# jteutenberg/downpore

Measured on AMD Instinct MI355X. Metric: overlaps/sec (all-vs-all PAF), higher is better.
Workload: dtype u64

## Files before the change

downpore_amd/csrc/dp_kbuild.hip:

```cpp
#include <algorithm>
#include <cstdio>
#include <cstdlib>
#include <cstring>

#include "dp_common.h"

typedef unsigned long long kb_u64;

#define KB_TILE 16384
#define KB_THREADS 1024
#define KB_P3_CAP 8192

struct KbGeom {
    int k, b1, b2, r;
    int pbits, rbits;
    uint32_t dlo, dhi;
};

struct KbBuf {
    uint32_t* lo;
    void* hi;
    int hb;
};
__device__ __forceinline__ kb_u64 kb_ld(const KbBuf B, kb_u64 i) {
    if (B.hb == 8) return ((const kb_u64*)B.lo)[i];
    kb_u64 v = B.lo[i];
    if (B.hb == 1) v |= (kb_u64)((const uint8_t*)B.hi)[i] << 32;
    else if (B.hb == 2) v |= (kb_u64)((const uint16_t*)B.hi)[i] << 32;
    else if (B.hb == 4) v |= (kb_u64)((const uint32_t*)B.hi)[i] << 32;
    return v;
}
__device__ __forceinline__ void kb_st(const KbBuf B, kb_u64 i, kb_u64 v) {
    if (B.hb == 8) {
        ((kb_u64*)B.lo)[i] = v;
        return;
    }
    B.lo[i] = (uint32_t)v;
    if (B.hb == 1) ((uint8_t*)B.hi)[i] = (uint8_t)(v >> 32);
    else if (B.hb == 2) ((uint16_t*)B.hi)[i] = (uint16_t)(v >> 32);
    else if (B.hb == 4) ((uint32_t*)B.hi)[i] = (uint32_t)(v >> 32);
}

__global__ void kb_group_table(const uint64_t* __restrict__ boff, uint32_t n_reads, uint32_t* __restrict__ gread) {
    const uint32_t r = blockIdx.x * blockDim.x + threadIdx.x;
    if (r >= n_reads) return;
    const uint64_t a0 = boff[r] * 4, a1 = boff[r + 1] * 4;
    for (uint64_t j = (a0 + 1023) >> 10; (j << 10) < a1; j++) gread[j] = r;
}

__device__ __forceinline__ uint32_t kb_read_of(uint64_t a, const uint32_t* __restrict__ gread, const uint64_t* __restrict__ boff) {
    uint32_t r = gread[a >> 10];
    while (boff[r + 1] * 4 <= a) r++;
    return r;
}

__device__ __forceinline__ uint32_t kb_load16(const uint8_t* __restrict__ packed, const uint64_t* __restrict__ boff,
                                              const uint32_t* __restrict__ len, const uint32_t* __restrict__ gread, uint64_t n_groups,
                                              uint64_t g, int half, int k, uint32_t kmer[16], uint32_t* read_out = nullptr,
                                              uint64_t* start_out = nullptr) {
    if (g >= n_groups) return 0u;
    const uint64_t a = g * 32 + (uint64_t)half * 16;
    const uint32_t r = kb_read_of(g * 32, gread, boff);
    const uint32_t L = len[r];
    if (L < (uint32_t)k) return 0u;
    const uint64_t a0 = boff[r] * 4, a1 = a0 + (L - k + 1);
    if (read_out) *read_out = r;
    if (start_out) *start_out = a0;
    if (a >= a1) return 0u;
    const uint32_t* p = (const uint32_t*)(packed + g * 8) + half;
    const uint32_t w0 = __builtin_bswap32(p[0]), w1 = __builtin_bswap32(p[1]);
    const int sh = 32 - 2 * k;
    uint32_t mask = 0;
#pragma unroll
    for (int j = 0; j < 16; j++) {
        const uint32_t win = j ? __builtin_amdgcn_alignbit(w0, w1, 32 - 2 * j) : w0;
        kmer[j] = win >> sh;
        if (a + j >= a0 && a + j < a1) mask |= 1u << j;
    }
    return mask;
}

__global__ __launch_bounds__(KB_THREADS) void kb_count1(const uint8_t* __restrict__ packed, const uint64_t* __restrict__ boff,
                                                        const uint32_t* __restrict__ len, const uint32_t* __restrict__ gread,
                                                        uint64_t n_groups, KbGeom G, kb_u64* __restrict__ cnt1) {
    __shared__ uint32_t hist[1024];
    const int nb = 1 << G.b1;
    for (int i = threadIdx.x; i < nb; i += KB_THREADS) hist[i] = 0;
    __syncthreads();
    const int dsh = 2 * G.k - G.b1;
    const uint64_t tiles = (n_groups * 2 + KB_THREADS - 1) / KB_THREADS;
    for (uint64_t t = blockIdx.x; t < tiles; t += gridDim.x) {
        const uint64_t h = t * KB_THREADS + threadIdx.x;
        uint32_t kmer[16];
        const uint32_t m = kb_load16(packed, boff, len, gread, n_groups, h >> 1, (int)(h & 1), G.k, kmer);
#pragma unroll
        for (int j = 0; j < 16; j++)
            if ((m >> j) & 1) atomicAdd(&hist[kmer[j] >> dsh], 1u);
    }
    __syncthreads();
    for (int i = threadIdx.x; i < nb; i += KB_THREADS)
        if (hist[i]) atomicAdd(&cnt1[i], (kb_u64)hist[i]);
}

template <int E>
__device__ __forceinline__ void kb_tile_out(const kb_u64 (&e)[E], uint32_t m, int dshift, uint32_t dmask, uint32_t* hist ,
                                            uint32_t* lstart , kb_u64* gbase , kb_u64* sorted ,
                                            kb_u64* __restrict__ cursor, const KbBuf out) {
    const int nb = (int)dmask + 1;
    for (int i = threadIdx.x; i < nb; i += KB_THREADS) hist[i] = 0;
    __syncthreads();
    uint32_t rk[E];
#pragma unroll
    for (int j = 0; j < E; j++) rk[j] = ((m >> j) & 1) ? atomicAdd(&hist[(uint32_t)(e[j] >> dshift) & dmask], 1u) : 0u;
    __syncthreads();
    {
        const int per = (nb + KB_THREADS - 1) / KB_THREADS;
        uint32_t loc[4] = {0, 0, 0, 0}, s = 0;
        for (int u = 0; u < per; u++) {
            const int b = threadIdx.x * per + u;
            loc[u] = b < nb ? hist[b] : 0u;
            s += loc[u];
        }
        const int lane = dp_lane(), wave = threadIdx.x >> 6;
        __shared__ uint32_t wsum[KB_THREADS / 64];
        uint32_t x = (uint32_t)wave_incl_sum((int)s);
        if (lane == 63) wsum[wave] = x;
        __syncthreads();
        uint32_t base = x - s;
        for (int w = 0; w < wave; w++) base += wsum[w];
        for (int u = 0; u < per; u++) {
            const int b = threadIdx.x * per + u;
            if (b < nb) {
                lstart[b] = base;
                if (loc[u]) gbase[b] = atomicAdd(&cursor[b], (kb_u64)loc[u]);
                base += loc[u];
            }
        }
    }
    __syncthreads();
    uint32_t total = 0;
#pragma unroll
    for (int j = 0; j < E; j++)
        if ((m >> j) & 1) {
            const uint32_t d = (uint32_t)(e[j] >> dshift) & dmask;
            sorted[lstart[d] + rk[j]] = e[j];
        }
    __syncthreads();
    total = lstart[nb - 1] + hist[nb - 1];
    for (uint32_t i = threadIdx.x; i < total; i += KB_THREADS) {
        const kb_u64 v = sorted[i];
        const uint32_t d = (uint32_t)(v >> dshift) & dmask;
        kb_st(out, gbase[d] + (kb_u64)(i - lstart[d]), v);
    }
    __syncthreads();
}

__global__ __launch_bounds__(KB_THREADS) void kb_part1(const uint8_t* __restrict__ packed, const uint64_t* __restrict__ boff,
                                                       const uint32_t* __restrict__ len, const uint32_t* __restrict__ gread,
                                                       uint64_t n_groups, KbGeom G, kb_u64* __restrict__ cursor, const KbBuf out) {
    __shared__ uint32_t hist[1024], lstart[1024];
    __shared__ kb_u64 gbase[1024];
    __shared__ kb_u64 sorted[KB_TILE];
    const int pay = G.pbits + G.rbits;
    const int dsh = pay + 2 * G.k - G.b1;
    const uint32_t dmask = (1u << G.b1) - 1u;
    const uint64_t tiles = (n_groups * 2 + KB_THREADS - 1) / KB_THREADS;
    for (uint64_t t = blockIdx.x; t < tiles; t += gridDim.x) {
        const uint64_t h = t * KB_THREADS + threadIdx.x;
        uint32_t kmer[16], rd = 0;
        uint64_t a0 = 0;
        const uint32_t m = kb_load16(packed, boff, len, gread, n_groups, h >> 1, (int)(h & 1), G.k, kmer, &rd, &a0);
        kb_u64 e[16];
        const kb_u64 a = (h >> 1) * 32 + (h & 1) * 16;
        const kb_u64 low = ((kb_u64)rd << G.pbits) + (a - a0);
        uint32_t mine = m;
        const int ksh = 2 * G.k - G.b1;
#pragma unroll
        for (int j = 0; j < 16; j++) {
            e[j] = ((kb_u64)kmer[j] << pay) | (low + (kb_u64)j);
            const uint32_t d = kmer[j] >> ksh;
            if (d < G.dlo || d >= G.dhi) mine &= ~(1u << j);
        }
        kb_tile_out<16>(e, mine, dsh, dmask, hist, lstart, gbase, sorted, cursor, out);
    }
}

__device__ __forceinline__ uint32_t kb_bucket_of_tile(const uint32_t* __restrict__ tile_start, int nb1, uint32_t t) {
    int lo = 0, hi = nb1;
    while (hi - lo > 1) {
        const int mid = (lo + hi) >> 1;
        if (tile_start[mid] <= t) lo = mid;
        else hi = mid;
    }
    return (uint32_t)lo;
}

__global__ __launch_bounds__(KB_THREADS) void kb_count2(const KbBuf in, const kb_u64* __restrict__ base1,
                                                        const uint32_t* __restrict__ tile_start, KbGeom G, kb_u64* __restrict__ cnt2) {
    __shared__ uint32_t hist[1024];
    const int nb1 = 1 << G.b1, nb2 = 1 << G.b2;
    const uint32_t n_tiles = tile_start[nb1];
    const int dsh = G.pbits + G.rbits + 2 * G.k - G.b1 - G.b2;
    const uint32_t dmask = (uint32_t)nb2 - 1u;
    for (uint32_t t = blockIdx.x; t < n_tiles; t += gridDim.x) {
        const uint32_t b = kb_bucket_of_tile(tile_start, nb1, t);
        const kb_u64 lo = base1[b] + (kb_u64)(t - tile_start[b]) * KB_TILE, hi = min(base1[b + 1], lo + KB_TILE);
        for (int i = threadIdx.x; i < nb2; i += KB_THREADS) hist[i] = 0;
        __syncthreads();
        for (kb_u64 i = lo + threadIdx.x; i < hi; i += KB_THREADS) atomicAdd(&hist[(uint32_t)(kb_ld(in, i) >> dsh) & dmask], 1u);
        __syncthreads();
        for (int i = threadIdx.x; i < nb2; i += KB_THREADS)
            if (hist[i]) atomicAdd(&cnt2[(kb_u64)b * nb2 + i], (kb_u64)hist[i]);
        __syncthreads();
    }
}

__global__ __launch_bounds__(KB_THREADS) void kb_part2(const KbBuf in, const kb_u64* __restrict__ base1,
                                                       const uint32_t* __restrict__ tile_start, KbGeom G, kb_u64* __restrict__ cursor2,
                                                       const KbBuf out) {
    __shared__ uint32_t hist[1024], lstart[1024];
    __shared__ kb_u64 gbase[1024];
    __shared__ kb_u64 sorted[KB_TILE];
    const int nb1 = 1 << G.b1, nb2 = 1 << G.b2;
    const uint32_t n_tiles = tile_start[nb1];
    const int dsh = G.pbits + G.rbits + 2 * G.k - G.b1 - G.b2;
    const uint32_t dmask = (uint32_t)nb2 - 1u;
    for (uint32_t t = blockIdx.x; t < n_tiles; t += gridDim.x) {
        const uint32_t b = kb_bucket_of_tile(tile_start, nb1, t);
        const kb_u64 lo = base1[b] + (kb_u64)(t - tile_start[b]) * KB_TILE, hi = min(base1[b + 1], lo + KB_TILE);
        kb_u64 e[KB_TILE / KB_THREADS];
        uint32_t m = 0;
#pragma unroll
        for (int j = 0; j < KB_TILE / KB_THREADS; j++) {
            const kb_u64 i = lo + (kb_u64)j * KB_THREADS + threadIdx.x;
            e[j] = 0;
            if (i < hi) {
                e[j] = kb_ld(in, i);
                m |= 1u << j;
            }
        }
        kb_tile_out<KB_TILE / KB_THREADS>(e, m, dsh, dmask, hist, lstart, gbase, sorted, cursor2 + (kb_u64)b * nb2, out);
    }
}

struct KbPosOut {
    void* lo;
    uint8_t* hi;
    int fmt;
};
__device__ __forceinline__ void kb_pos_st(const KbPosOut P, kb_u64 i, kb_u64 v, const KbGeom& G) {
    const kb_u64 pay = v & (((kb_u64)1 << (G.pbits + G.rbits)) - 1);
    if (P.fmt == 8) {
        ((kb_u64*)P.lo)[i] = ((pay >> G.pbits) << 32) | (pay & (((kb_u64)1 << G.pbits) - 1));
    } else {
        ((uint32_t*)P.lo)[i] = (uint32_t)pay;
        if (P.fmt == 5) P.hi[i] = (uint8_t)(pay >> 32);
    }
}
__global__ __launch_bounds__(KB_THREADS) void kb_final(const KbBuf in, const kb_u64* __restrict__ base2, uint32_t n_sub,
                                                       KbGeom G, const uint32_t* __restrict__ gread, const uint64_t* __restrict__ boff,
                                                       uint32_t* __restrict__ counts, kb_u64* __restrict__ off, const KbPosOut pos) {
    extern __shared__ kb_u64 kb_dyn[];
    const int nb = 1 << G.r;
    kb_u64* sorted = kb_dyn;
    uint32_t* hist = (uint32_t*)(kb_dyn + KB_P3_CAP);
    uint32_t* lstart = hist + nb;
    const uint32_t dmask = (uint32_t)nb - 1u;
    const int pay = G.pbits + G.rbits;
    for (uint32_t sp = blockIdx.x; sp < n_sub; sp += gridDim.x) {
        const kb_u64 lo = base2[sp], hi = base2[sp + 1];
        const kb_u64 n = hi - lo;
        for (int i = threadIdx.x; i < nb; i += KB_THREADS) hist[i] = 0;
        __syncthreads();
        constexpr int KB_HOLD = KB_P3_CAP / KB_THREADS;
        kb_u64 held[KB_HOLD];
        uint32_t rk[KB_HOLD];
        const bool hold = n <= KB_P3_CAP;
        if (hold) {
#pragma unroll
            for (int u = 0; u < KB_HOLD; u++) {
                const kb_u64 i = lo + (kb_u64)u * KB_THREADS + threadIdx.x;
                held[u] = i < hi ? kb_ld(in, i) : 0;
                rk[u] = i < hi ? atomicAdd(&hist[(uint32_t)(held[u] >> pay) & dmask], 1u) : 0u;
            }
        } else {
            for (kb_u64 i = lo + threadIdx.x; i < hi; i += KB_THREADS) atomicAdd(&hist[(uint32_t)(kb_ld(in, i) >> pay) & dmask], 1u);
        }
        __syncthreads();
        {
            const int per = (nb + KB_THREADS - 1) / KB_THREADS;
            uint32_t s = 0;
            for (int u = 0; u < per; u++) {
                const int b = threadIdx.x * per + u;
                if (b < nb) s += hist[b];
            }
            const int lane = dp_lane(), wave = threadIdx.x >> 6;
            __shared__ uint32_t wsum[KB_THREADS / 64];
            uint32_t x = (uint32_t)wave_incl_sum((int)s);
            if (lane == 63) wsum[wave] = x;
            __syncthreads();
            uint32_t base = x - s;
            for (int w = 0; w < wave; w++) base += wsum[w];
            for (int u = 0; u < per; u++) {
                const int b = threadIdx.x * per + u;
                if (b < nb) {
                    lstart[b] = base;
                    base += hist[b];
                }
            }
        }
        __syncthreads();
        const kb_u64 kbase = (kb_u64)sp << G.r;
        for (int b = threadIdx.x; b < nb; b += KB_THREADS) {
            counts[kbase + b] = hist[b];
            off[kbase + b] = lo + lstart[b];
        }
        if (hold) {
#pragma unroll
            for (int u = 0; u < KB_HOLD; u++) {
                const kb_u64 i = lo + (kb_u64)u * KB_THREADS + threadIdx.x;
                if (i < hi) {
                    const kb_u64 v = held[u];
                    const uint32_t d = (uint32_t)(v >> pay) & dmask;
                    sorted[lstart[d] + rk[u]] = v;
                }
            }
            __syncthreads();
            for (uint32_t i = threadIdx.x; i < (uint32_t)n; i += KB_THREADS) {
                kb_pos_st(pos, lo + i, sorted[i], G);
            }
        } else {
            __syncthreads();
            for (int i = threadIdx.x; i < nb; i += KB_THREADS) hist[i] = 0;
            __syncthreads();
            for (kb_u64 i = lo + threadIdx.x; i < hi; i += KB_THREADS) {
                const kb_u64 v = kb_ld(in, i);
                const uint32_t d = (uint32_t)(v >> pay) & dmask;
                kb_pos_st(pos, lo + lstart[d] + atomicAdd(&hist[d], 1u), v, G);
            }
        }
        __syncthreads();
    }
    if (blockIdx.x == 0 && threadIdx.x == 0) off[(kb_u64)n_sub << G.r] = base2[n_sub];
}

__global__ void kb_mask_digits(kb_u64* __restrict__ cnt1, uint32_t nb1, uint32_t dlo, uint32_t dhi) {
    const uint32_t d = blockIdx.x * blockDim.x + threadIdx.x;
    if (d < nb1 && (d < dlo || d >= dhi)) cnt1[d] = 0;
}

__global__ void kb_excl_scan_small(const kb_u64* __restrict__ in, uint32_t n, kb_u64* __restrict__ out) {
    __shared__ kb_u64 part[1024];
    const uint32_t per = (((n + 1023) / 1024) + 15u) & ~15u;
    const uint32_t lo = min(n, threadIdx.x * per), hi = min(n, lo + per);
    kb_u64 s = 0;
    for (uint32_t i = lo; i < hi; i += 16) {
        kb_u64 v[16];
#pragma unroll
        for (int j = 0; j < 16; j++) v[j] = i + j < hi ? in[i + j] : 0;
#pragma unroll
        for (int j = 0; j < 16; j++) s += v[j];
    }
    part[threadIdx.x] = s;
    __syncthreads();
    for (int d = 1; d < 1024; d <<= 1) {
        const kb_u64 v = (int)threadIdx.x >= d ? part[threadIdx.x - d] : 0;
        __syncthreads();
        part[threadIdx.x] += v;
        __syncthreads();
    }
    kb_u64 run = part[threadIdx.x] - s;
    for (uint32_t i = lo; i < hi; i += 16) {
        kb_u64 v[16];
#pragma unroll
        for (int j = 0; j < 16; j++) v[j] = i + j < hi ? in[i + j] : 0;
#pragma unroll
        for (int j = 0; j < 16; j++) {
            if (i + j < hi) out[i + j] = run;
            run += v[j];
        }
    }
    if (threadIdx.x == 1023) out[n] = run;
}

__global__ __launch_bounds__(1024) void kb_scan_partials(const kb_u64* __restrict__ in, uint32_t n, uint32_t chunk, kb_u64* __restrict__ partial) {
    __shared__ kb_u64 red[16];
    const uint32_t lo = min(n, blockIdx.x * chunk), hi = min(n, lo + chunk);
    kb_u64 s = 0;
    for (uint32_t i = lo + threadIdx.x; i < hi; i += 1024) s += in[i];
    for (int o = 32; o > 0; o >>= 1) s += __shfl_xor(s, o, 64);
    if (dp_lane() == 0) red[threadIdx.x >> 6] = s;
    __syncthreads();
    if (threadIdx.x == 0) {
        kb_u64 t = 0;
        for (int w = 0; w < 16; w++) t += red[w];
        partial[blockIdx.x] = t;
    }
}
__global__ __launch_bounds__(1024) void kb_scan_write(const kb_u64* __restrict__ in, uint32_t n, uint32_t chunk, const kb_u64* __restrict__ pbase,
                                                      kb_u64* __restrict__ out) {
    __shared__ kb_u64 part[1024];
    const uint32_t lo = min(n, blockIdx.x * chunk), hi = min(n, lo + chunk);
    kb_u64 run = pbase[blockIdx.x];
    for (uint32_t b0 = lo; b0 < hi; b0 += 1024) {
        const uint32_t i = b0 + threadIdx.x;
        const kb_u64 v = i < hi ? in[i] : 0;
        part[threadIdx.x] = v;
        __syncthreads();
        for (int d = 1; d < 1024; d <<= 1) {
            const kb_u64 u = (int)threadIdx.x >= d ? part[threadIdx.x - d] : 0;
            __syncthreads();
            part[threadIdx.x] += u;
            __syncthreads();
        }
        if (i < hi) out[i] = run + part[threadIdx.x] - v;
        run += part[1023];
        __syncthreads();
    }
    if (blockIdx.x == gridDim.x - 1 && threadIdx.x == 0) out[n] = run;
}

int dp_kindex_build_sorted(dp_ctx* ctx, dp_ctx* ow, int k, uint32_t* d_counts, uint64_t* d_off, void** d_pos_out, void** d_pos_hi_out,
                           int* fmt_out, int* pbits_out, uint64_t* n_pos_out, float* ms_out, dp_kindex_shard* shard) {
    if (k < 9 || k > 14 || ow->n_reads == 0) return 1;
    if (dp_tune("kindex_atomic", 0)) return 1;
    const uint64_t n_groups = (ow->packed_bytes * 4 + 31) / 32;
    KbGeom G;
    G.k = k;
    {
        uint32_t max_len = 1;
        for (uint32_t r = 0; r < ow->n_reads; r++) max_len = std::max(max_len, ow->h_len[r]);
        G.pbits = 1;
        while (((uint64_t)1 << G.pbits) <= max_len) G.pbits++;
        G.rbits = 1;
        while (((uint64_t)1 << G.rbits) < ow->n_reads) G.rbits++;
        if (const char* e = getenv("DP_KB_MIN_PBITS")) G.pbits = std::max(G.pbits, std::min(32, atoi(e)));
        if (2 * k + G.pbits + G.rbits > 64) return 1;
    }
    const int pay = G.pbits + G.rbits;
    G.b1 = 8;
    G.b1 = (int)std::max(6L, std::min(10L, dp_tune("kb_b1", G.b1)));
    if (G.b1 > 2 * k - 2) G.b1 = 2 * k - 2;
    const uint64_t approx = ow->total_bases;
    int b2 = std::max(1, 14 - G.b1);
    while (b2 < 10 && (approx >> (G.b1 + b2)) > 7800) b2++;
    if (G.b1 + b2 > 2 * k) b2 = 2 * k - G.b1;
    G.b2 = b2;
    G.r = 2 * k - G.b1 - G.b2;
    if (G.r > 12) {
        G.b2 += G.r - 12;
        G.r = 12;
    }
    if (G.b2 > 10) return 1;
    const int nb1 = 1 << G.b1, nb2 = 1 << G.b2;
    G.dlo = 0;
    G.dhi = (uint32_t)nb1;
    const uint32_t n_sub = (uint32_t)nb1 * (uint32_t)nb2;
    const bool wide = getenv("DP_KINDEX_WIDE") != nullptr;
    const int hb1 = 8, hb2 = 8;
    (void)wide;
    const int fmt = (wide || pay > 40) ? 8 : pay > 32 ? 5 : 4;
    const bool a_lo_wide = hb1 == 8 || fmt == 8;
    const bool f_over_a = a_lo_wide == (fmt == 8);
    {
        const uint64_t per_entry = (uint64_t)((a_lo_wide ? 8 : 4) + (hb1 != 8 ? hb1 : 0)) + (uint64_t)(hb2 == 8 ? 8 : 4 + hb2) + (f_over_a ? 0u : 4u) + (fmt == 5 ? 1u : 0u);
        size_t free_b = 0, total_b = 0;
        hipMemGetInfo(&free_b, &total_b);
        free_b += dp_dev_cached_bytes();
        const uint64_t mine = shard && shard->n_ranks > 1 ? ow->total_bases / (uint64_t)shard->n_ranks + (ow->total_bases >> 6) : ow->total_bases;
        if ((uint64_t)free_b < mine * per_entry + ((uint64_t)6 << 30)) return 1;
    }
    void *d_gread = nullptr, *d_small = nullptr, *d_a_lo = nullptr, *d_a_hi = nullptr, *d_b_lo = nullptr, *d_b_hi = nullptr, *d_f_hi = nullptr;
    struct Temps {
        std::vector<void**> v;
        ~Temps() {
            for (void** p : v)
                if (*p) dp_dev_free(*p);
        }
    } temps{{&d_gread, &d_small, &d_a_lo, &d_a_hi, &d_b_lo, &d_b_hi, &d_f_hi}};
    const size_t n_blocks1k = (size_t)((ow->packed_bytes * 4 + 1023) >> 10) + 2;
    DP_HIP(dp_dev_malloc(&d_gread, n_blocks1k * 4));
    const size_t small_u64 = (size_t)nb1 * 3 + 1 + (size_t)n_sub * 3 + 1;
    DP_HIP(dp_dev_malloc(&d_small, small_u64 * 8 + ((size_t)nb1 + 1) * 4 + 64));
    kb_u64* cnt1 = (kb_u64*)d_small;
    kb_u64* base1 = cnt1 + nb1;
    kb_u64* cur1 = base1 + nb1 + 1;
    kb_u64* cnt2 = cur1 + nb1;
    kb_u64* base2 = cnt2 + n_sub;
    kb_u64* cur2 = base2 + n_sub + 1;
    uint32_t* tile_start = (uint32_t*)(cur2 + n_sub);
    DP_HIP(hipMemsetAsync(d_small, 0, small_u64 * 8 + ((size_t)nb1 + 1) * 4, ctx->stream));
    hipEvent_t e0 = ctx->ev[2], e1 = ctx->ev[3];
    DP_HIP(hipEventRecord(e0, ctx->stream));
    hipLaunchKernelGGL(kb_group_table, dim3((ow->n_reads + 255) / 256), dim3(256), 0, ctx->stream, (const uint64_t*)ow->d_boff.p, ow->n_reads,
                       (uint32_t*)d_gread);
    int cus = 256;
    hipDeviceGetAttribute(&cus, hipDeviceAttributeMultiprocessorCount, ctx->device);
    const uint32_t grid = (uint32_t)cus * 8;
    hipLaunchKernelGGL(kb_count1, dim3(grid), dim3(KB_THREADS), 0, ctx->stream, (const uint8_t*)ow->d_packed.p, (const uint64_t*)ow->d_boff.p,
                       (const uint32_t*)ow->d_len.p, (const uint32_t*)d_gread, n_groups, G, cnt1);
    if (shard) {
        std::vector<kb_u64> h_cnt((size_t)nb1);
        DP_HIP(hipMemcpyAsync(h_cnt.data(), cnt1, (size_t)nb1 * 8, hipMemcpyDeviceToHost, ctx->stream));
        DP_HIP(dp_stream_sync(ctx));
        kb_u64 all = 0;
        for (int b = 0; b < nb1; b++) all += h_cnt[(size_t)b];
        const int N = shard->n_ranks;
        shard->digit_first.assign((size_t)N + 1, (uint32_t)nb1);
        shard->entry_first.assign((size_t)N + 1, all);
        std::vector<kb_u64> pre((size_t)nb1 + 1, 0);
        for (int b = 0; b < nb1; b++) pre[(size_t)b + 1] = pre[(size_t)b] + h_cnt[(size_t)b];
        shard->digit_first[0] = 0;
        shard->entry_first[0] = 0;
        for (int q = 1; q < N; q++) {
            const kb_u64 want = (all * (kb_u64)q + (kb_u64)N - 1) / (kb_u64)N;
            int b = (int)shard->digit_first[(size_t)q - 1];
            while (b < nb1 && pre[(size_t)b] < want) b++;
            shard->digit_first[(size_t)q] = (uint32_t)b;
            shard->entry_first[(size_t)q] = pre[(size_t)b];
        }
        shard->digit_first[(size_t)N] = (uint32_t)nb1;
        shard->entry_first[(size_t)N] = all;
        shard->kmer_shift = 2 * k - G.b1;
        shard->total = all;
        G.dlo = shard->digit_first[(size_t)shard->rank];
        G.dhi = shard->digit_first[(size_t)shard->rank + 1];
        hipLaunchKernelGGL(kb_mask_digits, dim3((nb1 + 255) / 256), dim3(256), 0, ctx->stream, cnt1, (uint32_t)nb1, G.dlo, G.dhi);
    }
    hipLaunchKernelGGL(kb_excl_scan_small, dim3(1), dim3(1024), 0, ctx->stream, (const kb_u64*)cnt1, (uint32_t)nb1, base1);
    DP_HIP(hipGetLastError());
    std::vector<kb_u64> h_base1((size_t)nb1 + 1);
    DP_HIP(hipMemcpyAsync(h_base1.data(), base1, ((size_t)nb1 + 1) * 8, hipMemcpyDeviceToHost, ctx->stream));
    DP_HIP(dp_stream_sync(ctx));
    const uint64_t n = h_base1[(size_t)nb1];
    std::vector<uint32_t> h_tiles((size_t)nb1 + 1);
    uint64_t tt = 0;
    for (int b = 0; b < nb1; b++) {
        h_tiles[(size_t)b] = (uint32_t)tt;
        tt += (h_base1[(size_t)b + 1] - h_base1[(size_t)b] + KB_TILE - 1) / KB_TILE;
    }
    h_tiles[(size_t)nb1] = (uint32_t)tt;
    if (tt >= 0xffffffffull) return 1;
    void* d_f_lo = nullptr;
    temps.v.push_back(&d_f_lo);
#define KB_ALLOC(p_, bytes_)                              \
    if (dp_dev_malloc(&(p_), (bytes_)) != hipSuccess) {   \
        (void)hipGetLastError();                          \
        return 1;                                         \
    }
    KB_ALLOC(d_a_lo, n * (size_t)(a_lo_wide ? 8 : 4) + 64)
    if (hb1 && hb1 != 8) KB_ALLOC(d_a_hi, n * (size_t)hb1 + 64)
    KB_ALLOC(d_b_lo, n * (size_t)(hb2 == 8 ? 8 : 4) + 64)
    if (hb2 && hb2 != 8) KB_ALLOC(d_b_hi, n * (size_t)hb2 + 64)
    if (fmt == 5) KB_ALLOC(d_f_hi, n + 64)
    if (!f_over_a) KB_ALLOC(d_f_lo, n * 4 + 64)
#undef KB_ALLOC
    const KbBuf A = {(uint32_t*)d_a_lo, d_a_hi, hb1}, B = {(uint32_t*)d_b_lo, d_b_hi, hb2};
    const KbPosOut F = {f_over_a ? d_a_lo : d_f_lo, (uint8_t*)d_f_hi, fmt};
    DP_HIP(hipMemcpyAsync(tile_start, h_tiles.data(), ((size_t)nb1 + 1) * 4, hipMemcpyHostToDevice, ctx->stream));
    DP_HIP(hipMemcpyAsync(cur1, base1, (size_t)nb1 * 8, hipMemcpyDeviceToDevice, ctx->stream));
    hipLaunchKernelGGL(kb_part1, dim3(grid), dim3(KB_THREADS), 0, ctx->stream, (const uint8_t*)ow->d_packed.p, (const uint64_t*)ow->d_boff.p,
                       (const uint32_t*)ow->d_len.p, (const uint32_t*)d_gread, n_groups, G, cur1, A);
    hipLaunchKernelGGL(kb_count2, dim3(grid), dim3(KB_THREADS), 0, ctx->stream, A, (const kb_u64*)base1, (const uint32_t*)tile_start, G, cnt2);
    if (n_sub >= 8192) {
        const uint32_t n_wg = 256, chunk = (((n_sub + n_wg - 1) / n_wg) + 1023u) & ~1023u;
        hipLaunchKernelGGL(kb_scan_partials, dim3(n_wg), dim3(1024), 0, ctx->stream, (const kb_u64*)cnt2, n_sub, chunk, cur2);
        hipLaunchKernelGGL(kb_excl_scan_small, dim3(1), dim3(1024), 0, ctx->stream, (const kb_u64*)cur2, n_wg, cur2 + n_wg);
        hipLaunchKernelGGL(kb_scan_write, dim3(n_wg), dim3(1024), 0, ctx->stream, (const kb_u64*)cnt2, n_sub, chunk, (const kb_u64*)(cur2 + n_wg), base2);
    } else {
        hipLaunchKernelGGL(kb_excl_scan_small, dim3(1), dim3(1024), 0, ctx->stream, (const kb_u64*)cnt2, n_sub, base2);
    }
    DP_HIP(hipMemcpyAsync(cur2, base2, (size_t)n_sub * 8, hipMemcpyDeviceToDevice, ctx->stream));
    hipLaunchKernelGGL(kb_part2, dim3(grid), dim3(KB_THREADS), 0, ctx->stream, A, (const kb_u64*)base1, (const uint32_t*)tile_start, G, cur2, B);
    hipLaunchKernelGGL(kb_final, dim3(std::min<uint32_t>(n_sub, (uint32_t)cus * 16)), dim3(KB_THREADS),
                       (size_t)KB_P3_CAP * 8 + ((size_t)8 << G.r), ctx->stream, B, (const kb_u64*)base2, n_sub, G, (const uint32_t*)d_gread,
                       (const uint64_t*)ow->d_boff.p, d_counts, (kb_u64*)d_off, F);
    DP_HIP(hipGetLastError());
    DP_HIP(hipEventRecord(e1, ctx->stream));
    DP_HIP(dp_stream_sync(ctx));
    if (ms_out) hipEventElapsedTime(ms_out, e0, e1);
    *d_pos_out = f_over_a ? d_a_lo : d_f_lo;
    (f_over_a ? d_a_lo : d_f_lo) = nullptr;
    *d_pos_hi_out = d_f_hi;
    d_f_hi = nullptr;
    *fmt_out = fmt;
    *pbits_out = G.pbits;
    *n_pos_out = n;
    return DP_OK;
}
```

Measured before the change: 40.70 million.

## Restructure k-mer bucket build: device-side bases, templated tiles, prefetch, grouped part2

Measured after the change: 41.69 million (median of 6 runs). 1.02x the previous value.

```diff
diff --git a/downpore_amd/csrc/dp_kbuild.hip b/downpore_amd/csrc/dp_kbuild.hip
--- a/downpore_amd/csrc/dp_kbuild.hip
+++ b/downpore_amd/csrc/dp_kbuild.hip
@@ -7,7 +7,7 @@
 
 typedef unsigned long long kb_u64;
 
-#define KB_TILE 16384
+#define KB_PER 16
 #define KB_THREADS 1024
 #define KB_P3_CAP 8192
 
@@ -54,28 +54,39 @@
     return r;
 }
 
-__device__ __forceinline__ uint32_t kb_load16(const uint8_t* __restrict__ packed, const uint64_t* __restrict__ boff,
-                                              const uint32_t* __restrict__ len, const uint32_t* __restrict__ gread, uint64_t n_groups,
-                                              uint64_t g, int half, int k, uint32_t kmer[16], uint32_t* read_out = nullptr,
-                                              uint64_t* start_out = nullptr) {
-    if (g >= n_groups) return 0u;
-    const uint64_t a = g * 32 + (uint64_t)half * 16;
+struct KbRaw {
+    uint32_t w0, w1, read;
+    uint64_t a, a0, a1;
+    bool any;
+};
+__device__ __forceinline__ KbRaw kb_fetch16(const uint8_t* __restrict__ packed, const uint64_t* __restrict__ boff,
+                                            const uint32_t* __restrict__ len, const uint32_t* __restrict__ gread, uint64_t n_groups,
+                                            uint64_t g, int half, int k) {
+    KbRaw R = {0u, 0u, 0u, g * 32 + (uint64_t)half * 16, 0, 0, false};
+    if (g >= n_groups) return R;
     const uint32_t r = kb_read_of(g * 32, gread, boff);
     const uint32_t L = len[r];
-    if (L < (uint32_t)k) return 0u;
-    const uint64_t a0 = boff[r] * 4, a1 = a0 + (L - k + 1);
-    if (read_out) *read_out = r;
-    if (start_out) *start_out = a0;
-    if (a >= a1) return 0u;
+    if (L < (uint32_t)k) return R;
+    R.read = r;
+    R.a0 = boff[r] * 4;
+    R.a1 = R.a0 + (L - k + 1);
+    if (R.a >= R.a1) return R;
     const uint32_t* p = (const uint32_t*)(packed + g * 8) + half;
-    const uint32_t w0 = __builtin_bswap32(p[0]), w1 = __builtin_bswap32(p[1]);
+    R.w0 = p[0];
+    R.w1 = p[1];
+    R.any = true;
+    return R;
+}
+__device__ __forceinline__ uint32_t kb_expand16(const KbRaw& R, int k, uint32_t kmer[16]) {
+    if (!R.any) return 0u;
+    const uint32_t w0 = __builtin_bswap32(R.w0), w1 = __builtin_bswap32(R.w1);
     const int sh = 32 - 2 * k;
     uint32_t mask = 0;
 #pragma unroll
     for (int j = 0; j < 16; j++) {
         const uint32_t win = j ? __builtin_amdgcn_alignbit(w0, w1, 32 - 2 * j) : w0;
         kmer[j] = win >> sh;
-        if (a + j >= a0 && a + j < a1) mask |= 1u << j;
+        if (R.a + j >= R.a0 && R.a + j < R.a1) mask |= 1u << j;
     }
     return mask;
 }
@@ -92,7 +103,7 @@
     for (uint64_t t = blockIdx.x; t < tiles; t += gridDim.x) {
         const uint64_t h = t * KB_THREADS + threadIdx.x;
         uint32_t kmer[16];
-        const uint32_t m = kb_load16(packed, boff, len, gread, n_groups, h >> 1, (int)(h & 1), G.k, kmer);
+        const uint32_t m = kb_expand16(kb_fetch16(packed, boff, len, gread, n_groups, h >> 1, (int)(h & 1), G.k), G.k, kmer);
 #pragma unroll
         for (int j = 0; j < 16; j++)
             if ((m >> j) & 1) atomicAdd(&hist[kmer[j] >> dsh], 1u);
@@ -102,19 +113,35 @@
         if (hist[i]) atomicAdd(&cnt1[i], (kb_u64)hist[i]);
 }
 
-template <int E>
-__device__ __forceinline__ void kb_tile_out(const kb_u64 (&e)[E], uint32_t m, int dshift, uint32_t dmask, uint32_t* hist ,
-                                            uint32_t* lstart , kb_u64* gbase , kb_u64* sorted ,
-                                            kb_u64* __restrict__ cursor, const KbBuf out) {
+template <int T>
+struct KbTileLds {
+    uint32_t hist[1024];
+    uint16_t lstart[1024];
+    kb_u64 gbase[1024];
+    uint32_t wsum[T / 64];
+    kb_u64 sorted[KB_PER * T];
+};
+struct KbNoPrefetch {
+    __device__ __forceinline__ void operator()() const {}
+};
+
+template <int T, class Prefetch>
+__device__ __forceinline__ void kb_tile_out(const kb_u64 (&e)[KB_PER], uint32_t m, int dshift, uint32_t dmask, KbTileLds<T>& S,
+                                            kb_u64* __restrict__ cursor, const KbBuf out, Prefetch&& prefetch) {
+    constexpr int E = KB_PER;
+    uint32_t* const hist = S.hist;
+    uint16_t* const lstart = S.lstart;
+    kb_u64* const gbase = S.gbase;
+    kb_u64* const sorted = S.sorted;
     const int nb = (int)dmask + 1;
-    for (int i = threadIdx.x; i < nb; i += KB_THREADS) hist[i] = 0;
+    for (int i = threadIdx.x; i < nb; i += T) hist[i] = 0;
     __syncthreads();
     uint32_t rk[E];
 #pragma unroll
     for (int j = 0; j < E; j++) rk[j] = ((m >> j) & 1) ? atomicAdd(&hist[(uint32_t)(e[j] >> dshift) & dmask], 1u) : 0u;
     __syncthreads();
     {
-        const int per = (nb + KB_THREADS - 1) / KB_THREADS;
+        const int per = (nb + T - 1) / T;
         uint32_t loc[4] = {0, 0, 0, 0}, s = 0;
         for (int u = 0; u < per; u++) {
             const int b = threadIdx.x * per + u;
@@ -122,7 +149,7 @@
             s += loc[u];
         }
         const int lane = dp_lane(), wave = threadIdx.x >> 6;
-        __shared__ uint32_t wsum[KB_THREADS / 64];
+        uint32_t* const wsum = S.wsum;
         uint32_t x = (uint32_t)wave_incl_sum((int)s);
         if (lane == 63) wsum[wave] = x;
         __syncthreads();
@@ -131,7 +158,7 @@
         for (int u = 0; u < per; u++) {
             const int b = threadIdx.x * per + u;
             if (b < nb) {
-                lstart[b] = base;
+                lstart[b] = (uint16_t)base;
                 if (loc[u]) gbase[b] = atomicAdd(&cursor[b], (kb_u64)loc[u]);
                 base += loc[u];
             }
@@ -146,8 +173,9 @@
             sorted[lstart[d] + rk[j]] = e[j];
         }
     __syncthreads();
+    prefetch();
     total = lstart[nb - 1] + hist[nb - 1];
-    for (uint32_t i = threadIdx.x; i < total; i += KB_THREADS) {
+    for (uint32_t i = threadIdx.x; i < total; i += T) {
         const kb_u64 v = sorted[i];
         const uint32_t d = (uint32_t)(v >> dshift) & dmask;
         kb_st(out, gbase[d] + (kb_u64)(i - lstart[d]), v);
@@ -155,24 +183,28 @@
     __syncthreads();
 }
 
-__global__ __launch_bounds__(KB_THREADS) void kb_part1(const uint8_t* __restrict__ packed, const uint64_t* __restrict__ boff,
-                                                       const uint32_t* __restrict__ len, const uint32_t* __restrict__ gread,
-                                                       uint64_t n_groups, KbGeom G, kb_u64* __restrict__ cursor, const KbBuf out) {
-    __shared__ uint32_t hist[1024], lstart[1024];
-    __shared__ kb_u64 gbase[1024];
-    __shared__ kb_u64 sorted[KB_TILE];
+template <int T, bool PRE>
+__global__ __launch_bounds__(T, T == 256 ? 3 : 4) void kb_part1(const uint8_t* __restrict__ packed, const uint64_t* __restrict__ boff,
+                                                 const uint32_t* __restrict__ len, const uint32_t* __restrict__ gread, uint64_t n_groups,
+                                                 KbGeom G, kb_u64* __restrict__ cursor, const KbBuf out, const uint32_t* __restrict__ bad) {
+    __shared__ KbTileLds<T> S;
+    if (*bad) return;
     const int pay = G.pbits + G.rbits;
     const int dsh = pay + 2 * G.k - G.b1;
     const uint32_t dmask = (1u << G.b1) - 1u;
-    const uint64_t tiles = (n_groups * 2 + KB_THREADS - 1) / KB_THREADS;
+    const uint64_t tiles = (n_groups * 2 + T - 1) / T;
+    auto fetch = [&](uint64_t t) {
+        const uint64_t h = t * T + threadIdx.x;
+        return kb_fetch16(packed, boff, len, gread, n_groups, h >> 1, (int)(h & 1), G.k);
+    };
+    KbRaw raw = {};
+    if (PRE) raw = fetch(blockIdx.x);
     for (uint64_t t = blockIdx.x; t < tiles; t += gridDim.x) {
-        const uint64_t h = t * KB_THREADS + threadIdx.x;
-        uint32_t kmer[16], rd = 0;
-        uint64_t a0 = 0;
-        const uint32_t m = kb_load16(packed, boff, len, gread, n_groups, h >> 1, (int)(h & 1), G.k, kmer, &rd, &a0);
+        if (!PRE) raw = fetch(t);
+        uint32_t kmer[16];
+        const uint32_t m = kb_expand16(raw, G.k, kmer);
         kb_u64 e[16];
-        const kb_u64 a = (h >> 1) * 32 + (h & 1) * 16;
-        const kb_u64 low = ((kb_u64)rd << G.pbits) + (a - a0);
+        const kb_u64 low = ((kb_u64)raw.read << G.pbits) + (raw.a - raw.a0);
         uint32_t mine = m;
         const int ksh = 2 * G.k - G.b1;
 #pragma unroll
@@ -181,7 +213,9 @@
             const uint32_t d = kmer[j] >> ksh;
             if (d < G.dlo || d >= G.dhi) mine &= ~(1u << j);
         }
-        kb_tile_out<16>(e, mine, dsh, dmask, hist, lstart, gbase, sorted, cursor, out);
+        kb_tile_out<T>(e, mine, dsh, dmask, S, cursor, out, [&] {
+            if (PRE) raw = fetch(t + gridDim.x);
+        });
     }
 }
 
@@ -196,15 +230,16 @@
 }
 
 __global__ __launch_bounds__(KB_THREADS) void kb_count2(const KbBuf in, const kb_u64* __restrict__ base1,
-                                                        const uint32_t* __restrict__ tile_start, KbGeom G, kb_u64* __restrict__ cnt2) {
+                                                        const uint32_t* __restrict__ tile_start, uint32_t tile, KbGeom G,
+                                                        kb_u64* __restrict__ cnt2, uint32_t b_lo, uint32_t b_hi) {
     __shared__ uint32_t hist[1024];
     const int nb1 = 1 << G.b1, nb2 = 1 << G.b2;
-    const uint32_t n_tiles = tile_start[nb1];
+    const uint32_t n_tiles = tile_start[b_hi];
     const int dsh = G.pbits + G.rbits + 2 * G.k - G.b1 - G.b2;
     const uint32_t dmask = (uint32_t)nb2 - 1u;
-    for (uint32_t t = blockIdx.x; t < n_tiles; t += gridDim.x) {
+    for (uint32_t t = tile_start[b_lo] + blockIdx.x; t < n_tiles; t += gridDim.x) {
         const uint32_t b = kb_bucket_of_tile(tile_start, nb1, t);
-        const kb_u64 lo = base1[b] + (kb_u64)(t - tile_start[b]) * KB_TILE, hi = min(base1[b + 1], lo + KB_TILE);
+        const kb_u64 lo = base1[b] + (kb_u64)(t - tile_start[b]) * tile, hi = min(base1[b + 1], lo + tile);
         for (int i = threadIdx.x; i < nb2; i += KB_THREADS) hist[i] = 0;
         __syncthreads();
         for (kb_u64 i = lo + threadIdx.x; i < hi; i += KB_THREADS) atomicAdd(&hist[(uint32_t)(kb_ld(in, i) >> dsh) & dmask], 1u);
@@ -215,31 +250,30 @@
     }
 }
 
-__global__ __launch_bounds__(KB_THREADS) void kb_part2(const KbBuf in, const kb_u64* __restrict__ base1,
-                                                       const uint32_t* __restrict__ tile_start, KbGeom G, kb_u64* __restrict__ cursor2,
-                                                       const KbBuf out) {
-    __shared__ uint32_t hist[1024], lstart[1024];
-    __shared__ kb_u64 gbase[1024];
-    __shared__ kb_u64 sorted[KB_TILE];
+template <int T>
+__global__ __launch_bounds__(T, T == 256 ? 3 : 4) void kb_part2(const KbBuf in, const kb_u64* __restrict__ base1, const uint32_t* __restrict__ tile_start,
+                                                 KbGeom G, kb_u64* __restrict__ cursor2, const KbBuf out, uint32_t b_lo, uint32_t b_hi) {
+    __shared__ KbTileLds<T> S;
+    constexpr uint32_t TILE = KB_PER * T;
     const int nb1 = 1 << G.b1, nb2 = 1 << G.b2;
-    const uint32_t n_tiles = tile_start[nb1];
+    const uint32_t n_tiles = tile_start[b_hi];
     const int dsh = G.pbits + G.rbits + 2 * G.k - G.b1 - G.b2;
     const uint32_t dmask = (uint32_t)nb2 - 1u;
-    for (uint32_t t = blockIdx.x; t < n_tiles; t += gridDim.x) {
+    for (uint32_t t = tile_start[b_lo] + blockIdx.x; t < n_tiles; t += gridDim.x) {
         const uint32_t b = kb_bucket_of_tile(tile_start, nb1, t);
-        const kb_u64 lo = base1[b] + (kb_u64)(t - tile_start[b]) * KB_TILE, hi = min(base1[b + 1], lo + KB_TILE);
-        kb_u64 e[KB_TILE / KB_THREADS];
+        const kb_u64 lo = base1[b] + (kb_u64)(t - tile_start[b]) * TILE, hi = min(base1[b + 1], lo + TILE);
+        kb_u64 e[KB_PER];
         uint32_t m = 0;
 #pragma unroll
-        for (int j = 0; j < KB_TILE / KB_THREADS; j++) {
-            const kb_u64 i = lo + (kb_u64)j * KB_THREADS + threadIdx.x;
+        for (int j = 0; j < KB_PER; j++) {
+            const kb_u64 i = lo + (kb_u64)j * T + threadIdx.x;
             e[j] = 0;
             if (i < hi) {
                 e[j] = kb_ld(in, i);
                 m |= 1u << j;
             }
         }
-        kb_tile_out<KB_TILE / KB_THREADS>(e, m, dsh, dmask, hist, lstart, gbase, sorted, cursor2 + (kb_u64)b * nb2, out);
+        kb_tile_out<T>(e, m, dsh, dmask, S, cursor2 + (kb_u64)b * nb2, out, KbNoPrefetch());
     }
 }
 
@@ -257,30 +291,52 @@
         if (P.fmt == 5) P.hi[i] = (uint8_t)(pay >> 32);
     }
 }
-__global__ __launch_bounds__(KB_THREADS) void kb_final(const KbBuf in, const kb_u64* __restrict__ base2, uint32_t n_sub,
-                                                       KbGeom G, const uint32_t* __restrict__ gread, const uint64_t* __restrict__ boff,
-                                                       uint32_t* __restrict__ counts, kb_u64* __restrict__ off, const KbPosOut pos) {
+template <int W, bool PRE>
+__global__ __launch_bounds__(KB_THREADS, W) void kb_final(const KbBuf in, const kb_u64* __restrict__ base2, uint32_t n_sub, KbGeom G,
+                                                          uint32_t* __restrict__ counts, kb_u64* __restrict__ off, const KbPosOut pos,
+                                                          const uint32_t* __restrict__ bad) {
     extern __shared__ kb_u64 kb_dyn[];
+    if (*bad) return;
     const int nb = 1 << G.r;
     kb_u64* sorted = kb_dyn;
     uint32_t* hist = (uint32_t*)(kb_dyn + KB_P3_CAP);
     uint32_t* lstart = hist + nb;
     const uint32_t dmask = (uint32_t)nb - 1u;
     const int pay = G.pbits + G.rbits;
-    for (uint32_t sp = blockIdx.x; sp < n_sub; sp += gridDim.x) {
-        const kb_u64 lo = base2[sp], hi = base2[sp + 1];
+    constexpr int KB_HOLD = KB_P3_CAP / KB_THREADS;
+    kb_u64 held[KB_HOLD];
+    auto load_held = [&](kb_u64 lo, kb_u64 hi) {
+        if (hi - lo > KB_P3_CAP) return;
+#pragma unroll
+        for (int u = 0; u < KB_HOLD; u++) {
+            const kb_u64 i = lo + (kb_u64)u * KB_THREADS + threadIdx.x;
+            held[u] = i < hi ? kb_ld(in, i) : 0;
+        }
+    };
+    uint32_t sp = blockIdx.x;
+    kb_u64 lo = 0, hi = 0;
+    if (sp < n_sub) {
+        lo = base2[sp];
+        hi = base2[sp + 1];
+        if (PRE) load_held(lo, hi);
+    }
+    while (sp < n_sub) {
         const kb_u64 n = hi - lo;
+        const uint32_t nsp = sp + gridDim.x;
+        kb_u64 nlo = 0, nhi = 0;
+        if (nsp < n_sub) {
+            nlo = base2[nsp];
+            nhi = base2[nsp + 1];
+        }
         for (int i = threadIdx.x; i < nb; i += KB_THREADS) hist[i] = 0;
         __syncthreads();
-        constexpr int KB_HOLD = KB_P3_CAP / KB_THREADS;
-        kb_u64 held[KB_HOLD];
         uint32_t rk[KB_HOLD];
         const bool hold = n <= KB_P3_CAP;
         if (hold) {
+            if (!PRE) load_held(lo, hi);
 #pragma unroll
             for (int u = 0; u < KB_HOLD; u++) {
                 const kb_u64 i = lo + (kb_u64)u * KB_THREADS + threadIdx.x;
-                held[u] = i < hi ? kb_ld(in, i) : 0;
                 rk[u] = i < hi ? atomicAdd(&hist[(uint32_t)(held[u] >> pay) & dmask], 1u) : 0u;
             }
         } else {
@@ -326,6 +382,7 @@
                 }
             }
             __syncthreads();
+            if (PRE) load_held(nlo, nhi);
             for (uint32_t i = threadIdx.x; i < (uint32_t)n; i += KB_THREADS) {
                 kb_pos_st(pos, lo + i, sorted[i], G);
             }
@@ -333,6 +390,7 @@
             __syncthreads();
             for (int i = threadIdx.x; i < nb; i += KB_THREADS) hist[i] = 0;
             __syncthreads();
+            if (PRE) load_held(nlo, nhi);
             for (kb_u64 i = lo + threadIdx.x; i < hi; i += KB_THREADS) {
                 const kb_u64 v = kb_ld(in, i);
                 const uint32_t d = (uint32_t)(v >> pay) & dmask;
@@ -340,6 +398,9 @@
             }
         }
         __syncthreads();
+        sp = nsp;
+        lo = nlo;
+        hi = nhi;
     }
     if (blockIdx.x == 0 && threadIdx.x == 0) off[(kb_u64)n_sub << G.r] = base2[n_sub];
 }
@@ -349,7 +410,38 @@
     if (d < nb1 && (d < dlo || d >= dhi)) cnt1[d] = 0;
 }
 
-__global__ void kb_excl_scan_small(const kb_u64* __restrict__ in, uint32_t n, kb_u64* __restrict__ out) {
+__global__ __launch_bounds__(1024) void kb_bases1(const kb_u64* __restrict__ cnt1, uint32_t nb1, uint32_t tile, kb_u64 n_expected,
+                                                  kb_u64* __restrict__ base1, kb_u64* __restrict__ cur1, uint32_t* __restrict__ tile_start,
+                                                  uint32_t* __restrict__ bad) {
+    __shared__ kb_u64 pe[1024], pt[1024];
+    const uint32_t i = threadIdx.x;
+    const kb_u64 c = i < nb1 ? cnt1[i] : 0, tl = (c + tile - 1) / tile;
+    pe[i] = c;
+    pt[i] = tl;
+    __syncthreads();
+    for (uint32_t d = 1; d < 1024; d <<= 1) {
+        const kb_u64 ve = i >= d ? pe[i - d] : 0, vt = i >= d ? pt[i - d] : 0;
+        __syncthreads();
+        pe[i] += ve;
+        pt[i] += vt;
+        __syncthreads();
+    }
+    const kb_u64 total = pe[1023], tiles = pt[1023];
+    const bool ok = total == n_expected && tiles < 0xffffffffull;
+    if (i < nb1) {
+        base1[i] = pe[i] - c;
+        cur1[i] = pe[i] - c;
+        tile_start[i] = ok ? (uint32_t)(pt[i] - tl) : 0u;
+    }
+    if (i == 0) {
+        base1[nb1] = total;
+        tile_start[nb1] = ok ? (uint32_t)tiles : 0u;
+        *bad = ok ? 0u : 1u;
+    }
+}
+
+__global__ void kb_excl_scan_small(const kb_u64* __restrict__ in, uint32_t n, kb_u64* __restrict__ out, kb_u64* __restrict__ out2,
+                                   const kb_u64* __restrict__ init) {
     __shared__ kb_u64 part[1024];
     const uint32_t per = (((n + 1023) / 1024) + 15u) & ~15u;
     const uint32_t lo = min(n, threadIdx.x * per), hi = min(n, lo + per);
@@ -369,14 +461,17 @@
         part[threadIdx.x] += v;
         __syncthreads();
     }
-    kb_u64 run = part[threadIdx.x] - s;
+    kb_u64 run = part[threadIdx.x] - s + (init ? *init : 0);
     for (uint32_t i = lo; i < hi; i += 16) {
         kb_u64 v[16];
 #pragma unroll
         for (int j = 0; j < 16; j++) v[j] = i + j < hi ? in[i + j] : 0;
 #pragma unroll
         for (int j = 0; j < 16; j++) {
-            if (i + j < hi) out[i + j] = run;
+            if (i + j < hi) {
+                out[i + j] = run;
+                if (out2) out2[i + j] = run;
+            }
             run += v[j];
         }
     }
@@ -398,7 +493,7 @@
     }
 }
 __global__ __launch_bounds__(1024) void kb_scan_write(const kb_u64* __restrict__ in, uint32_t n, uint32_t chunk, const kb_u64* __restrict__ pbase,
-                                                      kb_u64* __restrict__ out) {
+                                                      kb_u64* __restrict__ out, kb_u64* __restrict__ out2) {
     __shared__ kb_u64 part[1024];
     const uint32_t lo = min(n, blockIdx.x * chunk), hi = min(n, lo + chunk);
     kb_u64 run = pbase[blockIdx.x];
@@ -413,7 +508,7 @@
             part[threadIdx.x] += u;
             __syncthreads();
         }
-        if (i < hi) out[i] = run + part[threadIdx.x] - v;
+        if (i < hi) out[i] = out2[i] = run + part[threadIdx.x] - v;
         run += part[1023];
         __syncthreads();
     }
@@ -470,26 +565,53 @@
         const uint64_t mine = shard && shard->n_ranks > 1 ? ow->total_bases / (uint64_t)shard->n_ranks + (ow->total_bases >> 6) : ow->total_bases;
         if ((uint64_t)free_b < mine * per_entry + ((uint64_t)6 << 30)) return 1;
     }
-    void *d_gread = nullptr, *d_small = nullptr, *d_a_lo = nullptr, *d_a_hi = nullptr, *d_b_lo = nullptr, *d_b_hi = nullptr, *d_f_hi = nullptr;
+    const int t1 = (int)dp_tune("kb_t1", 512), t2 = (int)dp_tune("kb_t2", 1024);
+    const bool pre1 = dp_tune("kb_pre1", 0) != 0, pre3 = dp_tune("kb_pre3", 0) != 0, occ3 = dp_tune("kb_occ3", 1) != 0;
+    const int grp2 = (int)dp_tune("kb_grp2", 0);
+    if ((t1 != 256 && t1 != 512 && t1 != 1024) || (t2 != 256 && t2 != 512 && t2 != 1024)) return 1;
+    const uint32_t tile2 = (uint32_t)(KB_PER * t2);
+    uint64_t n = 0;
+    for (uint32_t r = 0; r < ow->n_reads; r++) n += ow->h_len[r] >= (uint32_t)k ? ow->h_len[r] - (uint32_t)k + 1 : 0;
+    void *d_gread = nullptr, *d_small = nullptr, *d_a_lo = nullptr, *d_a_hi = nullptr, *d_b_lo = nullptr, *d_b_hi = nullptr, *d_f_hi = nullptr,
+         *d_f_lo = nullptr;
     struct Temps {
         std::vector<void**> v;
         ~Temps() {
             for (void** p : v)
                 if (*p) dp_dev_free(*p);
         }
-    } temps{{&d_gread, &d_small, &d_a_lo, &d_a_hi, &d_b_lo, &d_b_hi, &d_f_hi}};
+    } temps{{&d_gread, &d_small, &d_a_lo, &d_a_hi, &d_b_lo, &d_b_hi, &d_f_hi, &d_f_lo}};
+    auto alloc_entries = [&]() -> bool {
+        if (n / tile2 + (uint64_t)nb1 >= 0xffffffffull) return false;
+        auto get = [&](void*& p_, size_t bytes_) {
+            if (dp_dev_malloc(&p_, bytes_) == hipSuccess) return true;
+            (void)hipGetLastError();
+            return false;
+        };
+        if (!get(d_a_lo, n * (size_t)(a_lo_wide ? 8 : 4) + 64)) return false;
+        if (hb1 && hb1 != 8 && !get(d_a_hi, n * (size_t)hb1 + 64)) return false;
+        if (!get(d_b_lo, n * (size_t)(hb2 == 8 ? 8 : 4) + 64)) return false;
+        if (hb2 && hb2 != 8 && !get(d_b_hi, n * (size_t)hb2 + 64)) return false;
+        if (fmt == 5 && !get(d_f_hi, n + 64)) return false;
+        if (!f_over_a && !get(d_f_lo, n * 4 + 64)) return false;
+        return true;
+    };
     const size_t n_blocks1k = (size_t)((ow->packed_bytes * 4 + 1023) >> 10) + 2;
     DP_HIP(dp_dev_malloc(&d_gread, n_blocks1k * 4));
-    const size_t small_u64 = (size_t)nb1 * 3 + 1 + (size_t)n_sub * 3 + 1;
-    DP_HIP(dp_dev_malloc(&d_small, small_u64 * 8 + ((size_t)nb1 + 1) * 4 + 64));
+    const uint32_t n_wg = 256;
+    const size_t small_u64 = (size_t)nb1 * 3 + 1 + (size_t)n_sub * 3 + 1 + 2 * n_wg + 1, small_u32 = (size_t)nb1 + 2;
+    DP_HIP(dp_dev_malloc(&d_small, small_u64 * 8 + small_u32 * 4 + 64));
     kb_u64* cnt1 = (kb_u64*)d_small;
     kb_u64* base1 = cnt1 + nb1;
     kb_u64* cur1 = base1 + nb1 + 1;
     kb_u64* cnt2 = cur1 + nb1;
     kb_u64* base2 = cnt2 + n_sub;
     kb_u64* cur2 = base2 + n_sub + 1;
-    uint32_t* tile_start = (uint32_t*)(cur2 + n_sub);
-    DP_HIP(hipMemsetAsync(d_small, 0, small_u64 * 8 + ((size_t)nb1 + 1) * 4, ctx->stream));
+    kb_u64* partial = cur2 + n_sub;
+    uint32_t* tile_start = (uint32_t*)(partial + 2 * n_wg + 1);
+    uint32_t* bad = tile_start + nb1 + 1;
+    if (!shard && !alloc_entries()) return 1;
+    DP_HIP(hipMemsetAsync(d_small, 0, small_u64 * 8 + small_u32 * 4, ctx->stream));
     hipEvent_t e0 = ctx->ev[2], e1 = ctx->ev[3];
     DP_HIP(hipEventRecord(e0, ctx->stream));
     hipLaunchKernelGGL(kb_group_table, dim3((ow->n_reads + 255) / 256), dim3(256), 0, ctx->stream, (const uint64_t*)ow->d_boff.p, ow->n_reads,
@@ -526,58 +648,74 @@
         G.dlo = shard->digit_first[(size_t)shard->rank];
         G.dhi = shard->digit_first[(size_t)shard->rank + 1];
         hipLaunchKernelGGL(kb_mask_digits, dim3((nb1 + 255) / 256), dim3(256), 0, ctx->stream, cnt1, (uint32_t)nb1, G.dlo, G.dhi);
-    }
-    hipLaunchKernelGGL(kb_excl_scan_small, dim3(1), dim3(1024), 0, ctx->stream, (const kb_u64*)cnt1, (uint32_t)nb1, base1);
-    DP_HIP(hipGetLastError());
-    std::vector<kb_u64> h_base1((size_t)nb1 + 1);
-    DP_HIP(hipMemcpyAsync(h_base1.data(), base1, ((size_t)nb1 + 1) * 8, hipMemcpyDeviceToHost, ctx->stream));
-    DP_HIP(dp_stream_sync(ctx));
-    const uint64_t n = h_base1[(size_t)nb1];
-    std::vector<uint32_t> h_tiles((size_t)nb1 + 1);
-    uint64_t tt = 0;
-    for (int b = 0; b < nb1; b++) {
-        h_tiles[(size_t)b] = (uint32_t)tt;
-        tt += (h_base1[(size_t)b + 1] - h_base1[(size_t)b] + KB_TILE - 1) / KB_TILE;
-    }
-    h_tiles[(size_t)nb1] = (uint32_t)tt;
-    if (tt >= 0xffffffffull) return 1;
-    void* d_f_lo = nullptr;
-    temps.v.push_back(&d_f_lo);
-#define KB_ALLOC(p_, bytes_)                              \
-    if (dp_dev_malloc(&(p_), (bytes_)) != hipSuccess) {   \
-        (void)hipGetLastError();                          \
-        return 1;                                         \
-    }
-    KB_ALLOC(d_a_lo, n * (size_t)(a_lo_wide ? 8 : 4) + 64)
-    if (hb1 && hb1 != 8) KB_ALLOC(d_a_hi, n * (size_t)hb1 + 64)
-    KB_ALLOC(d_b_lo, n * (size_t)(hb2 == 8 ? 8 : 4) + 64)
-    if (hb2 && hb2 != 8) KB_ALLOC(d_b_hi, n * (size_t)hb2 + 64)
-    if (fmt == 5) KB_ALLOC(d_f_hi, n + 64)
-    if (!f_over_a) KB_ALLOC(d_f_lo, n * 4 + 64)
-#undef KB_ALLOC
+        n = pre[(size_t)G.dhi] - pre[(size_t)G.dlo];
+        if (!alloc_entries()) return 1;
+    }
     const KbBuf A = {(uint32_t*)d_a_lo, d_a_hi, hb1}, B = {(uint32_t*)d_b_lo, d_b_hi, hb2};
     const KbPosOut F = {f_over_a ? d_a_lo : d_f_lo, (uint8_t*)d_f_hi, fmt};
-    DP_HIP(hipMemcpyAsync(tile_start, h_tiles.data(), ((size_t)nb1 + 1) * 4, hipMemcpyHostToDevice, ctx->stream));
-    DP_HIP(hipMemcpyAsync(cur1, base1, (size_t)nb1 * 8, hipMemcpyDeviceToDevice, ctx->stream));
-    hipLaunchKernelGGL(kb_part1, dim3(grid), dim3(KB_THREADS), 0, ctx->stream, (const uint8_t*)ow->d_packed.p, (const uint64_t*)ow->d_boff.p,
-                       (const uint32_t*)ow->d_len.p, (const uint32_t*)d_gread, n_groups, G, cur1, A);
-    hipLaunchKernelGGL(kb_count2, dim3(grid), dim3(KB_THREADS), 0, ctx->stream, A, (const kb_u64*)base1, (const uint32_t*)tile_start, G, cnt2);
-    if (n_sub >= 8192) {
-        const uint32_t n_wg = 256, chunk = (((n_sub + n_wg - 1) / n_wg) + 1023u) & ~1023u;
-        hipLaunchKernelGGL(kb_scan_partials, dim3(n_wg), dim3(1024), 0, ctx->stream, (const kb_u64*)cnt2, n_sub, chunk, cur2);
-        hipLaunchKernelGGL(kb_excl_scan_small, dim3(1), dim3(1024), 0, ctx->stream, (const kb_u64*)cur2, n_wg, cur2 + n_wg);
-        hipLaunchKernelGGL(kb_scan_write, dim3(n_wg), dim3(1024), 0, ctx->stream, (const kb_u64*)cnt2, n_sub, chunk, (const kb_u64*)(cur2 + n_wg), base2);
+    hipLaunchKernelGGL(kb_bases1, dim3(1), dim3(1024), 0, ctx->stream, (const kb_u64*)cnt1, (uint32_t)nb1, tile2, (kb_u64)n, base1, cur1, tile_start,
+                       bad);
+#define KB_PART1(T_, PRE_)                                                                                                                  \
+    hipLaunchKernelGGL((kb_part1<T_, PRE_>), dim3(grid), dim3(T_), 0, ctx->stream, (const uint8_t*)ow->d_packed.p, (const uint64_t*)ow->d_boff.p, \
+                       (const uint32_t*)ow->d_len.p, (const uint32_t*)d_gread, n_groups, G, cur1, A, (const uint32_t*)bad)
+    if (t1 == 1024) {
+        if (pre1) KB_PART1(1024, true);
+        else KB_PART1(1024, false);
+    } else if (t1 == 512) {
+        if (pre1) KB_PART1(512, true);
+        else KB_PART1(512, false);
     } else {
-        hipLaunchKernelGGL(kb_excl_scan_small, dim3(1), dim3(1024), 0, ctx->stream, (const kb_u64*)cnt2, n_sub, base2);
-    }
-    DP_HIP(hipMemcpyAsync(cur2, base2, (size_t)n_sub * 8, hipMemcpyDeviceToDevice, ctx->stream));
-    hipLaunchKernelGGL(kb_part2, dim3(grid), dim3(KB_THREADS), 0, ctx->stream, A, (const kb_u64*)base1, (const uint32_t*)tile_start, G, cur2, B);
-    hipLaunchKernelGGL(kb_final, dim3(std::min<uint32_t>(n_sub, (uint32_t)cus * 16)), dim3(KB_THREADS),
-                       (size_t)KB_P3_CAP * 8 + ((size_t)8 << G.r), ctx->stream, B, (const kb_u64*)base2, n_sub, G, (const uint32_t*)d_gread,
-                       (const uint64_t*)ow->d_boff.p, d_counts, (kb_u64*)d_off, F);
+        if (pre1) KB_PART1(256, true);
+        else KB_PART1(256, false);
+    }
+#undef KB_PART1
+#define KB_PART2(T_, lo_, hi_)                                                                                                              \
+    hipLaunchKernelGGL((kb_part2<T_>), dim3(grid), dim3(T_), 0, ctx->stream, A, (const kb_u64*)base1, (const uint32_t*)tile_start, G, cur2, B, \
+                       (uint32_t)(lo_), (uint32_t)(hi_))
+    auto part2 = [&](int lo_, int hi_) {
+        if (t2 == 1024) KB_PART2(1024, lo_, hi_);
+        else if (t2 == 512) KB_PART2(512, lo_, hi_);
+        else KB_PART2(256, lo_, hi_);
+    };
+    if (grp2 <= 0) {
+        hipLaunchKernelGGL(kb_count2, dim3(grid), dim3(KB_THREADS), 0, ctx->stream, A, (const kb_u64*)base1, (const uint32_t*)tile_start, tile2, G, cnt2,
+                           0u, (uint32_t)nb1);
+        if (n_sub >= 8192) {
+            const uint32_t chunk = (((n_sub + n_wg - 1) / n_wg) + 1023u) & ~1023u;
+            hipLaunchKernelGGL(kb_scan_partials, dim3(n_wg), dim3(1024), 0, ctx->stream, (const kb_u64*)cnt2, n_sub, chunk, partial);
+            hipLaunchKernelGGL(kb_excl_scan_small, dim3(1), dim3(1024), 0, ctx->stream, (const kb_u64*)partial, n_wg, partial + n_wg, (kb_u64*)nullptr,
+                               (const kb_u64*)nullptr);
+            hipLaunchKernelGGL(kb_scan_write, dim3(n_wg), dim3(1024), 0, ctx->stream, (const kb_u64*)cnt2, n_sub, chunk, (const kb_u64*)(partial + n_wg),
+                               base2, cur2);
+        } else {
+            hipLaunchKernelGGL(kb_excl_scan_small, dim3(1), dim3(1024), 0, ctx->stream, (const kb_u64*)cnt2, n_sub, base2, cur2, (const kb_u64*)nullptr);
+        }
+        part2(0, nb1);
+    } else {
+        for (int lo_ = 0; lo_ < nb1; lo_ += grp2) {
+            const int hi_ = std::min(nb1, lo_ + grp2);
+            hipLaunchKernelGGL(kb_count2, dim3(grid), dim3(KB_THREADS), 0, ctx->stream, A, (const kb_u64*)base1, (const uint32_t*)tile_start, tile2, G,
+                               cnt2, (uint32_t)lo_, (uint32_t)hi_);
+            hipLaunchKernelGGL(kb_excl_scan_small, dim3(1), dim3(1024), 0, ctx->stream, (const kb_u64*)(cnt2 + (size_t)lo_ * nb2),
+                               (uint32_t)((hi_ - lo_) * nb2), base2 + (size_t)lo_ * nb2, cur2 + (size_t)lo_ * nb2, (const kb_u64*)(base1 + lo_));
+            part2(lo_, hi_);
+        }
+    }
+#undef KB_PART2
+#define KB_FINAL(W_, PRE_)                                                                                                                 \
+    hipLaunchKernelGGL((kb_final<W_, PRE_>), dim3(std::min<uint32_t>(n_sub, (uint32_t)cus * 16)), dim3(KB_THREADS),                          \
+                       (size_t)KB_P3_CAP * 8 + ((size_t)8 << G.r), ctx->stream, B, (const kb_u64*)base2, n_sub, G, d_counts, (kb_u64*)d_off, F, \
+                       (const uint32_t*)bad)
+    if (pre3) KB_FINAL(4, true);
+    else if (occ3) KB_FINAL(8, false);
+    else KB_FINAL(4, false);
+#undef KB_FINAL
     DP_HIP(hipGetLastError());
     DP_HIP(hipEventRecord(e1, ctx->stream));
+    uint32_t h_bad = 0;
+    DP_HIP(hipMemcpyAsync(&h_bad, bad, 4, hipMemcpyDeviceToHost, ctx->stream));
     DP_HIP(dp_stream_sync(ctx));
+    if (h_bad) return 1;
     if (ms_out) hipEventElapsedTime(ms_out, e0, e1);
     *d_pos_out = f_over_a ? d_a_lo : d_f_lo;
     (f_over_a ? d_a_lo : d_f_lo) = nullptr;
```
